# zeynelacikgoez/PyAudioLocalization

Measured on AMD Instinct MI355X. Metric: mic-pair GCC-PHAT correlations/s @44.1kHz·1s, higher is better.
Workload: dtype f64; 1 GPU; metric run: 64 frame(s)/step/GPU x 64 mics x 44100 samples @ 44100 Hz, 2016 pairs/frame, max_expected_delay=0.05; n=88199 = 89 x 991: prime-factor inverse, Rader row DFTs (cyclic convolutions of 990 points in LDS) + dense column DFTs; mics=64, samples=44100, pairs_per_frame=2016, fused_column_statistics=default, finishing_column_pass=default, rader_columns=default, gather=none, split=frames, parallelism=frames sharded over 1 GPU(s)

## Files before the change

pyaudiolocalization_amd/csrc/engine.h:

```cpp
#pragma once
#include <hip/hip_runtime.h>

#include <cstdarg>
#include <cstdint>
#include <cstdio>
#include <map>
#include <string>
#include <tuple>
#include <vector>

#include "../../include/pal_hip.h"
#include "fin_scratch.h"
#include "fft_core.h"
#include "pair_route.h"
#include "plan_geometry.h"
#include "peak_types.h"
#include "resample_math.h"

namespace pal {

struct FinArgs;

struct Conv {
  ConvGeom g;
// ... 179 lines not shown
  int solve_positions_dev(const pal_pair_record* d_tables, int B, int M, const int32_t* lengths, const double* mics, const double* calib,
                          const double* weights, const double* extra_starts, const pal_solve_params* prm, pal_position_record* out);
  int solve_positions_loss_dev(const pal_pair_record* d_tables, int B, int M, const int32_t* lengths, const double* mics, const double* calib,
                               const double* weights, const double* extra_starts, const pal_solve_params* prm, pal_position_record* out,
                               int loss, double f_scale, double* pair_weights);
  int solve_positions_impl(const pal_pair_record* d_tables, int B, int M, const int32_t* lengths, const double* mics, const double* calib,
                           const double* weights, const double* extra_starts, const pal_solve_params* prm, pal_position_record* out,
                           int loss, double f_scale, double* pair_weights);
  int tdoa_closure_dev(const pal_pair_record* d_tables, int B, int M, const int32_t* lengths, int32_t tol, int32_t min_votes, int32_t weight_mode,
                       int32_t* d_votes, int32_t* d_mic_closed, double* d_weights, pal_closure_frame* d_summary);
  int closure_check(int B, int M, const int32_t* lengths, int32_t tol, int32_t min_votes, int32_t weight_mode);
  int lag_votes(const int32_t* d_lag, int B, int M, int tol, int32_t* d_votes);
  int frames_check(const char* what, int B, int M, const int32_t* lengths, int32_t tol);
  int tdoa_consensus_dev(const pal_pair_record* d_tables, const int32_t* d_cand_k, const double* d_cand_h, int B, int M, int K,
                         const int32_t* lengths, int32_t tol, int32_t rounds, int32_t* d_sel, pal_pair_record* d_table_out,
                         pal_consensus_frame* d_summary);
  int consensus_check(int B, int M, int K, const int32_t* lengths, int32_t tol, int32_t rounds);
  int srp_strips_check(int B, int M, int L, int T, int W);
  int srp_strips_rows(const double* d_rows, int64_t nrows, int L, int T, int W, double* d_strips);
  int srp_map_check(int B, int M, int T, const double* mics, double fs, double c, const pal_srp_grid* grid, int K, int R, bool any_output,
                    bool peaks_out);
  int srp_map_dev(const double* d_strips, int B, int M, int T, const double* mics, double fs, double c, const pal_srp_grid* grid,
                  const double* d_pair_weights, int K, int R, double* d_power, pal_srp_peak* d_peaks, pal_srp_frame* d_summary);
  int srp_peaks_check(int B, const pal_srp_grid* grid, int K, int R);
  int srp_peaks_dev(const double* d_power, int B, const pal_srp_grid* grid, int K, int R, pal_srp_peak* d_peaks, pal_srp_frame* d_summary);
  int32_t* solve_idx = nullptr;
  int solve_idx_M = 0;
  std::vector<double> rs_win;
  std::vector<ResampleTap> rs_host;
  int rs_num_table = 0;
  double rs_ratio = 0;
  int peaks(const double* corr, size_t stride, int rows, int n, int n2, const pal_phat_params& prm,
            pal_pair_record* table, int32_t* ksel_multi, int slot, double* hsel_multi = nullptr);
  int peaks_setup(const double* corr, size_t stride, int rows, int n, int n2, const pal_phat_params& prm, int blocks, int grid_n2, int slot, PeakArgs& a);
  int peaks_finish(PeakArgs& a, int rows, pal_pair_record* table, int32_t* ksel_multi, int slot, double* hsel_multi = nullptr);
  int pfa_rows(const Plan& pl, const cd* permuted, const int4* quads, int G, cd* Y, hipStream_t on);
  int fin_setup(const Plan& pl, int rows, int nblk, int grid_rows, const pal_phat_params& prm, int n2, pal_pair_record* table,
                int* need, int slot, PeakArgs& a, struct FinArgs& fa, unsigned& nwg, int G);
  int rows_lean_group(const Plan& pl, const double* corr, size_t stride, int G, int rows, const pal_phat_params& prm, int n2,
                      pal_pair_record* table, int* need, int slot);
  int pfa_pair_group_fin(const Plan& pl, const cd* permuted, const int4* quads, int G, int rows, cd* Y, const int* zero_rows,
                         const pal_phat_params& prm, int n2, pal_pair_record* table, int* need, int slot,
                         double* corr = nullptr, size_t stride = 0);
  int pfa_pair_group_fused(const Plan& pl, const cd* permuted, const int4* quads, int G, int rows, cd* Y, double* corr, size_t stride,
                           const int* zero_rows, const pal_phat_params& prm, int n2, pal_pair_record* table, int32_t* ksel_multi, int slot,
                           double* hsel_multi = nullptr);
  bool pfa_forward_applies(const Plan& pl, int len) const;
  int pfa_forward_spectra(Plan& pl, const double* frames, size_t frame_stride, int rows, int len, cd* spectra, const int* flags);
  bool pfa_forward = true;
  bool fin_cols = true;
  unsigned fin_epoch[3] = {};
  FinKey fin_key[3];
  unsigned fin_wrap = kFinEpochWrap;
  bool fin_strip_on = true;
  int fin_giveup = 0;
  bool fuse_peaks = true;
};

struct ProfScope {
  Engine* e;
  int slot;
  hipEvent_t a = nullptr;
  hipStream_t on;
  ProfScope(Engine* eng, const char* name, hipStream_t s = nullptr) : e(eng), slot(-1), on(s ? s : eng->stream) {
    if (e->profiling && e->prof_gate) {
      slot = e->prof_slot(name);
      e->prof_begin(slot, &a, on);
    }
  }
  ~ProfScope() {
    if (slot >= 0) e->prof_end(slot, a, on);
  }
};

#define PAL_TRY(expr)                \
  do {                               \
    int _rc = (expr);                \
    if (_rc != PAL_OK) return _rc;   \
  } while (0)

#define PAL_HIP(expr) PAL_TRY(check((expr), #expr))

}
```

pyaudiolocalization_amd/csrc/pal_api.hip:

```cpp
#include <dlfcn.h>

#include <cmath>
#include <cstring>

#include "closure_tiles.h"
#include "engine.h"

namespace pal {

static std::string g_create_error;

int Engine::fail(int code, const char* fmt, ...) {
  char buf[512];
  va_list ap;
  va_start(ap, fmt);
  vsnprintf(buf, sizeof buf, fmt, ap);
  va_end(ap);
  err = buf;
  return code;
}

int Engine::check(hipError_t e, const char* what) {
  if (e == hipSuccess) return PAL_OK;
  const int code = e == hipErrorOutOfMemory ? PAL_ERR_NOMEM : PAL_ERR_HIP;
// ... 277 lines not shown
      (rc = hipEventCreateWithFlags(&e->ev_join2, hipEventDisableTiming)) != hipSuccess ||
      (rc = hipEventCreateWithFlags(&e->ev_join3, hipEventDisableTiming)) != hipSuccess ||
      (rc = hipEventCreateWithFlags(&e->ev_fin, hipEventDisableTiming)) != hipSuccess) {
    g_create_error = std::string("device init: ") + hipGetErrorString(rc);
    delete e;
    return PAL_ERR_HIP;
  }
  {
    int cus = 0;
    if (hipDeviceGetAttribute(&cus, hipDeviceAttributeMultiprocessorCount, device) == hipSuccess && cus > 0) e->cu_count = cus;
  }
  const char* env = getenv("PAL_CHUNK");
  if (env && atoi(env) > 0) { e->chunk = atoi(env); e->chunk_auto = false; }
  env = getenv("PAL_OVERLAP");
  e->one_stream = env && atoi(env) == 0;
  env = getenv("PAL_RADIX3");
  if (env) e->plan_sw.allow_r3 = atoi(env) != 0;
  env = getenv("PAL_PFA");
  if (env) e->plan_sw.allow_pfa = atoi(env) != 0;
  env = getenv("PAL_RADER");
  if (env) e->plan_sw.allow_rader = atoi(env) != 0;
  env = getenv("PAL_PFA_BIG");
  if (env) e->plan_sw.allow_big = atoi(env) != 0;
  env = getenv("PAL_FOUR_REG");
  if (env) e->plan_sw.four_reg = atoi(env) != 0;
  env = getenv("PAL_XCD_ROWS");
  if (env) e->xcd_rows = atoi(env) != 0;
  env = getenv("PAL_ROWS_SHARED");
  if (env) e->rows_shared = atoi(env) != 0;
  env = getenv("PAL_PFA_FWD");
  if (env) e->pfa_forward = atoi(env) != 0;
  env = getenv("PAL_FUSED");
  if (env) e->fuse_peaks = atoi(env) != 0;
  env = getenv("PAL_R89");
  if (env) e->plan_sw.allow_r89 = atoi(env) != 0;
  env = getenv("PAL_FIN_SERIAL");
  if (env) e->fin_serial = atoi(env) != 0;
  env = getenv("PAL_FIN");
  if (env) e->fin_cols = atoi(env) != 0;
  env = getenv("PAL_ROWS_LEAN");
  if (env) e->rows_lean = atoi(env) != 0;
  env = getenv("PAL_PAIR_BLOCK");
  if (env) e->pair_block = atoi(env);
  env = getenv("PAL_ROWS_LEAN_MIN");
  if (env && atoll(env) >= 1) e->rows_lean_min = atoll(env);
  env = getenv("PAL_LEAN_STORE");
  if (env) e->lean_store = atoi(env) != 0;
  env = getenv("PAL_DEBUG_MEMO");
  if (env) e->debug_memo = atoi(env);
  env = getenv("PAL_DEBUG_FIN_WRAP");
  if (env && atoi(env) >= 2) e->fin_wrap = unsigned(atoi(env));
  env = getenv("PAL_FIN_STRIP");
  if (env) e->fin_strip_on = atoi(env) != 0;
  env = getenv("PAL_DEBUG_FIN_GIVEUP");
  if (env) e->fin_giveup = atoi(env) != 0 ? 1 : 0;
  env = getenv("PAL_MAX_PLANS");
  if (env && atoi(env) >= 2) e->max_plans = atoi(env);
  *out = reinterpret_cast<pal_handle>(e);
  return PAL_OK;
}

void pal_destroy(pal_handle h) {
  if (!h) return;
  Engine* e = reinterpret_cast<Engine*>(h);
  hipSetDevice(e->device);
  pal_comm_destroy(h);
  (void)e->clear_plans();
  for (cd* p : e->stage_tw) if (p) hipFree(p);
  for (cd* p : e->stage_twc) if (p) hipFree(p);
  for (void* p : e->ws) if (p) hipFree(p);
  if (e->quads) hipFree(e->quads);
  if (e->quads_blk) hipFree(e->quads_blk);
  if (e->perm_blk) hipFree(e->perm_blk);
  if (e->solve_idx) hipFree(e->solve_idx);
  for (hipEvent_t ev : e->ev_pool) hipEventDestroy(ev);
  hipStreamDestroy(e->stream2);
  hipStreamDestroy(e->stream3);
  hipEventDestroy(e->ev_fork);
  hipEventDestroy(e->ev_join2);
  hipEventDestroy(e->ev_join3);
  hipEventDestroy(e->ev_fin);
  hipStreamDestroy(e->stream);
  delete e;
}

const char* pal_last_error(pal_handle h) {
  if (!h) return g_create_error.c_str();
  return reinterpret_cast<Engine*>(h)->err.c_str();
}

#define ENGINE(h)                                   \
  if (!(h)) return PAL_ERR_INVALID;                 \
  Engine* e = reinterpret_cast<Engine*>(h);         \
  if (hipSetDevice(e->device) != hipSuccess) return e->fail(PAL_ERR_HIP, "hipSetDevice(%d) failed", e->device)

int pal_synchronize(pal_handle h) {
  ENGINE(h);
  PAL_TRY(e->check(hipStreamSynchronize(e->stream), "stream sync"));
  if (e->profiling) e->prof_flush();
  return check_status(e);
}

int pal_clear_plans(pal_handle h) {
  ENGINE(h);
  return e->clear_plans();
}
// ... 639 lines not shown
```

pyaudiolocalization_amd/csrc/pfa.hip:

```cpp
#include <cmath>
#include <cstdlib>
#include <vector>

#include "pfa_kernels.h"
#include "pfa_rader.h"
#include "pfa_cols_stats.h"
#include "pfa_cols_fin.h"
#include "pfa_forward.h"
#include "pfa_big.h"

namespace pal {

#ifndef PAL_BIG13_PTS
#define PAL_BIG13_PTS 32
#endif
#ifndef PAL_BIG14_PTS
#define PAL_BIG14_PTS 32
#endif
constexpr int kBig13 = PAL_BIG13_PTS, kBig14 = PAL_BIG14_PTS;

static_assert(kColChunk == kPfaTC && kColUnroll == kPfaUnr && kRader89 == kR89, "plan_geometry.h against the column pass's constants");
static_assert(sizeof(RowStep) == sizeof(int2) && sizeof(Cplx) == sizeof(cd), "plan_geometry.h tables are uploaded as they are");

void Engine::free_pfa(Pfa& f) {
// ... 186 lines not shown
                      int* need, int slot, PeakArgs& a, FinArgs& fa, unsigned& nwg, int G) {
  const int n = pl.n;
  PAL_TRY(peaks_setup(nullptr, 0, rows, n, n2, prm, nblk, 0, slot, a));
  const FinLayout lay = fin_layout(pair_group(n), nblk, grid_rows);
  char* base = nullptr;
  PAL_TRY(scratch(fin_scratch_slot(slot), lay.total, &base));
  PAL_TRY(status_words(&fa.status));
  fa.table = table;
  fa.need = need;
  fa.done = reinterpret_cast<unsigned*>(base);
  FinKey key;
  key.gmax = pair_group(n);
  key.nblk = nblk;
  key.grid_rows = grid_rows;
  key.block = ws_bytes[fin_scratch_slot(slot)];
  if (fin_must_zero(fin_key[slot], key, fin_epoch[slot], fin_wrap)) {
    PAL_HIP(hipMemsetAsync(base, 0, key.block, stream_of(slot)));
    fin_key[slot] = key;
    fin_epoch[slot] = 0;
  }
  fa.epoch = ++fin_epoch[slot];
  fa.emax = reinterpret_cast<double*>(base + lay.off_emax);
  fa.parts = reinterpret_cast<FinPartial*>(base + lay.off_parts);
  fa.edge = reinterpret_cast<double*>(base + lay.off_edge);
  fa.giveup = fin_giveup;
  fa.pw = 1;
  fa.corr = nullptr;
  fa.stride = 0;
  fa.store_rows = 0;
  fa.strip = nullptr;
  fa.st = fin_no_strip();
  fa.grid = nullptr;
  fa.roots = nullptr;
  fa.zero_rows = nullptr;
  fa.windowed = std::isnan(prm.max_expected_delay) ? 0 : 1;
  fa.win_lo = 1;
  fa.win_hi = n - 2;
  if (fa.windowed) {
    const double med = prm.max_expected_delay, fs = prm.fs;
    long long k = -1;
    if (med >= 0) {
      const double est = med * fs;
      k = est < double(n) ? (long long)est + 2 : (long long)n;
      while (k >= 0 && !(std::fabs(double(k) / fs) <= med)) --k;
    }
    if (k < 0) { fa.win_lo = 1; fa.win_hi = 0; }
    else {
      const long long lo = (long long)(n2 - 1) - k, hi = (long long)(n2 - 1) + k;
      fa.win_lo = int(lo < 1 ? 1 : lo);
      fa.win_hi = int(hi > n - 2 ? n - 2 : hi);
    }
  }
  fa.cheb = a.method == 0 && nohist(prm.threshold_method, prm.threshold_multiplier) ? 1 : 0;
  nwg = 8u * unsigned((G + 7) / 8) * unsigned(nblk);
  return PAL_OK;
}

int Engine::rows_lean_group(const Plan& pl, const double* corr, size_t stride, int G, int rows, const pal_phat_params& prm, int n2,
                            pal_pair_record* table, int* need, int slot) {
  constexpr int NS = 22;
  const hipStream_t on = stream_of(slot);
  const int chunks = (pl.n + kColsOwn - 1) / kColsOwn;
  const int nblk = (chunks + 4 * NS - 1) / (4 * NS);
  PeakArgs a;
  FinArgs fa;
  unsigned nwg = 0;
  PAL_TRY(fin_setup(pl, rows, nblk, 1, prm, n2, table, need, slot, a, fa, nwg, G));
  fa.pw = 4;
  fa.corr = const_cast<double*>(corr);
  fa.stride = stride;
  ProfScope ps(this, "k_rows_lean", on);
  k_rows_lean<NS><<<dim3(nwg), dim3(256), 0, on>>>(corr, stride, G, nblk, a, fa, rows);
  PAL_HIP(hipGetLastError());
  return PAL_OK;
}

int Engine::pfa_pair_group_fin(const Plan& pl, const cd* permuted, const int4* quads, int G, int rows, cd* Y, const int* zero_rows,
                               const pal_phat_params& prm, int n2, pal_pair_record* table, int* need, int slot,
                               double* corr, size_t stride) {
  const Pfa& f = pl.pfa;
  const hipStream_t on = stream_of(slot);
  const bool shortcols = f.nch <= 1;
  const int nblk = fin_blocks(f.n2, f.nch);
  PeakArgs a;
  FinArgs fa;
  unsigned nwg = 0;
  PAL_TRY(fin_setup(pl, rows, nblk, f.n1, prm, n2, table, need, slot, a, fa, nwg, G));
  fa.corr = corr;
  fa.stride = stride;
  fa.store_rows = corr ? 1 : 0;
  PAL_TRY(pfa_rows(pl, permuted, quads, G, Y, on));
  {
    ProfScope ps(this, corr ? "k_pfa_cols_lean" : "k_pfa_cols_fin", on);
    const dim3 grid(nwg);
    const bool full = (f.n1 - 1) / 2 == f.nch * kPfaTC;
    const bool hist = !(a.method > 0 || fa.cheb);
    const int nw = f.nch == 2 ? 2 : (f.nch == 3 && !hist ? 3 : 4);
    FinSrc src{Y, f.T, static_cast<const Rader89Tab*>(f.r89_tab)};
    const FinStrip st = fin_strip(pl.n, fa.windowed != 0, fa.win_lo, fa.win_hi, a.snr_w, !corr && !hist, fin_strip_on);
    if (st.on()) {
      PAL_TRY(scratch(fin_strip_slot(slot), size_t(2 * pair_group(pl.n)) * size_t(st.len) * sizeof(double), &fa.strip));
      fa.st = st;
      fa.grid = Y;
      fa.roots = f.r1;
      fa.zero_rows = zero_rows;
    }
    const bool strip = fa.strip != nullptr;
    PAL_TRY(fin_serialize(on));
#define PAL_COLS_FIN(MODE, HI, FU, NW) do { \
      if (!HI && strip) k_pfa_cols_fin<MODE, kPfaTC, kPfaUnr, HI, FU, NW, !HI><<<grid, dim3(64 * NW), 0, on>>>(src, f.n1, f.n2, G, f.nch, nblk, zero_rows, a, fa, rows); \
      else k_pfa_cols_fin<MODE, kPfaTC, kPfaUnr, HI, FU, NW, false><<<grid, dim3(64 * NW), 0, on>>>(src, f.n1, f.n2, G, f.nch, nblk, zero_rows, a, fa, rows); } while (0)
#define PAL_COLS_FIN_FU(MODE, HI, NW) do { if (full) PAL_COLS_FIN(MODE, HI, true, NW); else PAL_COLS_FIN(MODE, HI, false, NW); } while (0)
    if (!hist) fa.pw = shortcols ? 4 : nw;
    if (shortcols) { if (hist) PAL_COLS_FIN(kColsStrips, true, false, 4); else PAL_COLS_FIN(kColsStrips, false, false, 4); }
    else if (f.r89 && full && nw == 4) { if (hist) PAL_COLS_FIN(kColsRader89, true, true, 4); else PAL_COLS_FIN(kColsRader89, false, true, 4); }
    else if (nw == 3) PAL_COLS_FIN_FU(kColsDense, false, 3);
    else if (nw == 2) { if (hist) PAL_COLS_FIN_FU(kColsDense, true, 2); else PAL_COLS_FIN_FU(kColsDense, false, 2); }
    else { if (hist) PAL_COLS_FIN_FU(kColsDense, true, 4); else PAL_COLS_FIN_FU(kColsDense, false, 4); }
#undef PAL_COLS_FIN_FU
#undef PAL_COLS_FIN
    PAL_HIP(hipGetLastError());
    PAL_TRY(fin_done(on));
  }
  return PAL_OK;
}

}
```

pyaudiolocalization_amd/csrc/pfa_cols_fin.h:

```cpp
#pragma once
#include <climits>

#include "fin_scratch.h"
#include "pair_route.h"
#include "pfa_cols_stats.h"
#include "reduce.h"
#include "wave_reduce.h"

namespace pal {

struct FinPartial {
  double vmin, hb, plat;
  double s1, s2, a1;
  double hw, platw;
  double hm;
  double w1, w2;
  int mb, mw, mm, pad;
};
static_assert(sizeof(FinPartial) == 104 && sizeof(FinPartial) == kFinPartialBytes, "thirteen words (fin_scratch.h)");

struct FinArgs {
  pal_pair_record* table;
  int* need;
  unsigned* done;
  double* edge;
  double* emax;
  unsigned epoch;
  int giveup;
  FinPartial* parts;
  int* status;
  int win_lo, win_hi;
  int windowed;
  int pw;
  double* corr;
  size_t stride;
  int store_rows;
  int cheb;
  double* strip;
  FinStrip st;
  const cd* grid;
  const cd* roots;
  const int* zero_rows;
};

struct FinWave {
  double vmax, hb, hw, hm, plat, platw, nvmin, s1, s2, a1, w1, w2;
  int imax, mb, mw, mm;
};

struct FinShared {
  unsigned hwin[2 * kWin];
  int swin0[144];
  FinWave wave[4];
};
static_assert(sizeof(FinShared) <= 2 * (kLogBins + 1) * sizeof(unsigned), "the finish scratch aliases the histograms");
// ... 250 lines not shown
      atomicAdd(&fs.hwin[kWin + 1], ld_agent(&bh[q].total));
    }
    for (int e = tid; e < S * kWin && have; e += LANES) {
      const int q = e / kWin, k = e - q * kWin;
      const int b = fs.swin0[q] + k;
      const unsigned v = ld_agent(&bh[q].h[k]);
      if (b < w0) atomicAdd(&fs.hwin[kWin], v);
      else if (b < wend) atomicAdd(&fs.hwin[b - w0], v);
    }
    __syncthreads();
    const unsigned total = fs.hwin[kWin + 1], base = fs.hwin[kWin];
    have = have && w0 < wend && total == unsigned(n) && r1 >= base;
    double b1lo = 0, b1hi = 0, b2lo = 0, b2hi = 0;
    if (have) {
      unsigned e = base;
      int f1 = -1, f2 = -1;
      for (int k = 0; k < wend - w0; ++k) {
        const unsigned v = fs.hwin[k];
        if (f1 < 0 && r1 < e + v) f1 = k;
        if (f2 < 0 && r2 < e + v) f2 = k;
        e += v;
      }
      have = f1 >= 0 && f2 >= 0;
      if (have) {
        b1lo = log_bin_floor(w0 + f1); b1hi = log_bin_floor(w0 + f1 + 1);
        b2lo = log_bin_floor(w0 + f2); b2hi = log_bin_floor(w0 + f2 + 1);
      }
    }
    __syncthreads();
    if (have) {
      const double ml_ = r2 != r1 ? (b1lo + b2lo) * 0.5 : b1lo, mh_ = r2 != r1 ? (b1hi + b2hi) * 0.5 : b1hi;
      tlo = pa.mult >= 0 ? pa.mult * ml_ : pa.mult * mh_;
      thi = pa.mult >= 0 ? pa.mult * mh_ : pa.mult * ml_;
    } else {
      flag = true;
      why |= 16;
    }
  }
  fin_decide(pa, fa, row, s, flag, why, interval, tlo, thi, tid == 0);
}

}
#include "pfa_fin_lean.h"
namespace pal {

enum { kColsDense = 0, kColsRader89 = 1, kColsStrips = 2 };

struct FinSrc {
  const cd* Y;
  const double* T;
  const Rader89Tab* tab;
};

template <int MODE, int TC, int UNR, bool HIST, bool FULL, int NW, bool STRIP = false>
__global__ __launch_bounds__(64 * NW) __attribute__((amdgpu_waves_per_eu(MODE == kColsRader89 ? 3 : 2))) void k_pfa_cols_fin(FinSrc src, int N1, int N2, int G, int nch, int nblk,
                                                      const int* __restrict__ zero_rows, PeakArgs pa, FinArgs fa, int rows) {
  constexpr bool R89 = MODE == kColsRader89, STRIPS = MODE == kColsStrips;
  static_assert(!R89 || (NW == 4 && FULL), "the Rader column transform is the four-wavefront N1 = 89 case");
  static_assert(!HIST || NW <= 4, "the histogram form merges at most four wavefronts per block");
  static_assert(!(HIST && STRIP), "the strip form belongs to the per-wavefront statistics");
  const cd* __restrict__ Y = src.Y;
  const double* __restrict__ T = src.T;
  const Rader89Tab* __restrict__ tab = src.tab;
  constexpr int kHistDoubles = (2 * (kLogBins + 1) * int(sizeof(unsigned)) + 7) / 8;
  __shared__ __attribute__((aligned(16))) double lds_big[R89 ? 88 * 64 : kHistDoubles];
  unsigned (*const hist)[kLogBins + 1] = reinterpret_cast<unsigned (*)[kLogBins + 1]>(lds_big);
  __shared__ FinPartial res[4][2];
  __shared__ double wmax[4][2];
  __shared__ unsigned wtot[4][2];
  __shared__ int medbin[2];
  __shared__ int s_imax[2];
  __shared__ int s_flag;
  const int tid = threadIdx.x, lane = tid & 63;
  const int wave = __builtin_amdgcn_readfirstlane(tid >> 6);
  const int ch = STRIPS ? 0 : wave;
  const int xs = int(blockIdx.x & 7u), slot = int(blockIdx.x >> 3);
  const int cb = slot % nblk, g = xs + 8 * (slot / nblk);
  if (g >= G) return;
  const int strips = STRIPS ? nblk * NW : nblk, strip = STRIPS ? cb * NW + wave : cb;
  const int nact = STRIPS ? NW : nch;
  const int c_lo = int((long long)strip * N2 / strips), c_hi = int((long long)(strip + 1) * N2 / strips);
  const bool active = STRIPS ? true : ch < nch;
  const int m2 = c_lo - 1 + lane;
  const bool live = m2 >= 0 && m2 < N2 && lane <= c_hi - c_lo + 1;
  const bool own = live && lane >= 1 && lane <= c_hi - c_lo;
  const bool inner = own && m2 >= 1 && m2 <= N2 - 2;
  const int m2c = m2 < 0 ? 0 : (m2 < N2 ? m2 : N2 - 1);
  const int h = (N1 - 1) / 2;
  const int n = pa.n;
  constexpr bool want_median = HIST;
  constexpr int LANES = 64 * NW;
  if (want_median && !R89) {
    unsigned* hz = &hist[0][0];
    for (int q = tid; q < 2 * (kLogBins + 1); q += LANES) hz[q] = 0;
  }
  constexpr int TCD = R89 ? 1 : TC;
  double cx[TCD], sy[TCD], cy[TCD], sx[TCD];
  double sumx = 0, sumy = 0;
  cd y0 = mk(0, 0);
  cd ro[R89 ? kR89Slots : 1];
  cd c0 = mk(0, 0);
  const double kp = zero_rows && zero_rows[2 * g] ? 0.0 : 1.0, kq = zero_rows && 2 * g + 1 < rows && zero_rows[2 * g + 1] ? 0.0 : 1.0;
  int slot_t = 0;
  if constexpr (R89) {
    slot_t = tab->tmap[wave][lane < kR89Slots ? lane : 0];
    r89_columns(Y + size_t(g) * N1 * N2 + m2c, N2, wave, lane, tab, lds_big, ro, c0);
    if (want_median) {
      unsigned* hz = &hist[0][0];
      for (int q = tid; q < 2 * (kLogBins + 1); q += LANES) hz[q] = 0;
    }
    if (kp == 0.0 || kq == 0.0) {
      c0.x *= kp; c0.y *= kq;
#pragma unroll
      for (int i = 0; i < kR89Slots; ++i) { ro[i].x *= kp; ro[i].y *= kq; }
    }
  } else {
    if (active) pfa_cols_accumulate<TC, UNR>(Y + size_t(g) * N1 * N2 + m2c, N1, N2, nch, ch, T, y0, cx, sy, cy, sx, sumx, sumy);
    if (kp == 0.0) { y0.x = sumx = 0.0; }
    if (kq == 0.0) { y0.y = sumy = 0.0; }
#pragma unroll
    for (int tt = 0; tt < TCD; ++tt) {
      cx[tt] *= kp; sy[tt] *= kp; cy[tt] *= kq; sx[tt] *= kq;
    }
  }
  if constexpr (!HIST) {
    bool last;
    if constexpr (R89) {
      last = fin_lean_r89<true, false, kR89Slots, STRIP>(ro, c0, slot_t, 0u, wave, lane, g, cb, nblk, N1, N2, rows, c_lo, m2, own, inner, cb == 0 || cb == nblk - 1,
                                                  -1, true, pa, fa);
    } else {
// ... 368 lines not shown
```

pyaudiolocalization_amd/csrc/pfa_fin_lean.h:

```cpp
#pragma once

namespace pal {

__device__ __forceinline__ double wave_max63r(double v) { return wave_reduce_d(v, -__builtin_huge_val(), [](double a, double b) { return max_raw(a, b); }); }
__device__ __forceinline__ double wave_min63r(double v) { return wave_reduce_d(v, __builtin_huge_val(), [](double a, double b) { return min_raw(a, b); }); }
__device__ __forceinline__ double readlane_d(double v, int l) {
  return __hiloint2double(__builtin_amdgcn_readlane(__double2hiint(v), l), __builtin_amdgcn_readlane(__double2loint(v), l));
}

template <class BETTER> __device__ __forceinline__ void uniform_arg_sparse(double& v, int& i, BETTER better) {
  const unsigned long long cm = __ballot(i >= 0);
  if (cm == 0) { i = -1; v = 0; return; }
  if ((cm & (cm - 1)) == 0) {
    const int l = int(__builtin_ctzll(cm));
    v = readlane_d(v, l);
    i = __builtin_amdgcn_readlane(i, l);
    return;
  }
  wave_arg63(v, i, better);
  v = wave_bcast63(v);
  i = wave_bcast63(i);
}
__device__ __forceinline__ void uniform_arg_dense_hi(double& v, int& i) {
  const double h = wave_bcast63(wave_max63r(i >= 0 ? v : -__builtin_huge_val()));
// ... 2 lines not shown
  if ((tm & (tm - 1)) == 0) {
    i = __builtin_amdgcn_readlane(i, int(__builtin_ctzll(tm)));
  } else {
    int j = (i >= 0 && v == h) ? i : -1;
    j = wave_reduce_i(j, -1, [](int a, int b) { return a > b ? a : b; });
    i = wave_bcast63(j);
  }
  v = h;
}
__device__ __forceinline__ void uniform_arg_dense_lo(double& v, int& i) {
  const double h = wave_bcast63(wave_max63r(i >= 0 ? v : -__builtin_huge_val()));
  const unsigned long long tm = __ballot(i >= 0 && v == h);
  if (tm == 0) { i = -1; v = 0; return; }
  if ((tm & (tm - 1)) == 0) {
    i = __builtin_amdgcn_readlane(i, int(__builtin_ctzll(tm)));
  } else {
    int j = (i >= 0 && v == h) ? i : INT_MAX;
    j = wave_reduce_i(j, INT_MAX, [](int a, int b) { return a < b ? a : b; });
    i = wave_bcast63(j);
  }
  v = h;
}
__device__ __forceinline__ double uniform_max_sparse(double v) {
  if (__ballot(v > -__builtin_huge_val()) == 0) return -__builtin_huge_val();
  return wave_bcast63(wave_max63r(v));
}

constexpr int kQuadXor1 = 0xB1, kQuadXor2 = 0x4E, kRor4 = 0x124, kRor8 = 0x128;
template <class OP> __device__ __forceinline__ double wave_pair_reduce(double a, double b, OP op) {
  const bool odd = threadIdx.x & 1;
  double c = odd ? b : a;
  const double d = odd ? a : b;
  c = op(c, dpp_d<kQuadXor1>(0.0, d));
  c = op(c, dpp_d<kQuadXor2>(0.0, c));
  c = op(c, dpp_d<kRor4>(0.0, c));
  c = op(c, dpp_d<kRor8>(0.0, c));
  {
    const unsigned lo = unsigned(__double2loint(c)), hi = unsigned(__double2hiint(c));
    const auto l = __builtin_amdgcn_permlane16_swap(lo, lo, false, false);
    const auto h = __builtin_amdgcn_permlane16_swap(hi, hi, false, false);
    c = op(__hiloint2double(int(h[0]), int(l[0])), __hiloint2double(int(h[1]), int(l[1])));
  }
  {
    const unsigned lo = unsigned(__double2loint(c)), hi = unsigned(__double2hiint(c));
    const auto l = __builtin_amdgcn_permlane32_swap(lo, lo, false, false);
    const auto h = __builtin_amdgcn_permlane32_swap(hi, hi, false, false);
    c = op(__hiloint2double(int(h[0]), int(l[0])), __hiloint2double(int(h[1]), int(l[1])));
  }
  return c;
}
__device__ __forceinline__ double wave_pair_sum(double a, double b) { return wave_pair_reduce(a, b, [](double x, double y) { return x + y; }); }
__device__ __forceinline__ double wave_pair_min(double a, double b) { return wave_pair_reduce(a, b, [](double x, double y) { return min_raw(x, y); }); }

template <bool ALL, bool PART, int NS, bool STRIP = false>
__device__ __forceinline__ bool fin_lean_r89(const cd (&ro)[NS], const cd c0, const int slot_t, const unsigned emask, const int wave, const int lane,
                                             const int g, const int cb, const int nblk, const int N1, const int N2, const int rows, const int c_lo,
                                             const int m2, const bool own, const bool inner, const bool edge_block, const int pslot, const bool pvalid,
                                             const PeakArgs& pa, const FinArgs& fa) {
  static_assert(NS + 1 <= 32, "slot masks are 32 bits");
  static_assert(!(STRIP && PART), "row chunks read stored rows: their finisher reads the SNR window from the row");
  const int n = pa.n, S = pa.splits, PW = fa.pw;
  const unsigned long long pvm = PART ? __ballot(pvalid) : ~0ull;
  const unsigned long long ownm = __ballot(own), innerm = __ballot(inner);
  const int nrow = 2 * g + 1 < rows ? 2 : 1;
  const bool windowed = fa.windowed != 0;
  auto T = [&](int slot) { return slot == 0 ? 0 : __builtin_amdgcn_readlane(slot_t, slot - 1); };
  auto for_slots = [&](int r, auto&& fn) {
    if (ALL ? wave == 0 : (emask & 1u) != 0) fn(r ? c0.y : c0.x, 0);
#pragma unroll
    for (int i = 0; i < NS; ++i)
      if (ALL || (emask >> (i + 1) & 1u)) fn(r ? ro[i].y : ro[i].x, i + 1);
  };
  auto slot_mask = [&](int t_lo, int t_hi) -> unsigned {
    const unsigned long long b = __ballot(lane < NS && slot_t >= t_lo && slot_t <= t_hi);
    const unsigned m = (unsigned(b) << 1) | (t_lo <= 0 && t_hi >= 0 ? 1u : 0u);
    return ALL ? (wave == 0 ? m : m & ~1u) : m & emask;
  };
  int lo1 = 1, hi1 = 0;
  unsigned wmask = 0;
  if (windowed) {
    const int elo = fa.win_lo - (pa.dist - 1), ehi = fa.win_hi + (pa.dist - 1);
    lo1 = elo > 1 ? elo : 1;
    hi1 = ehi < n - 2 ? ehi : n - 2;
    if (lo1 <= hi1) wmask = slot_mask(lo1 / N2, hi1 / N2);
  }

  double vn[2], s1[2], s2[2], a1[2];
  FinPartial pt[2];
#pragma unroll
  for (int r = 0; r < 2; ++r) {
    vn[r] = INFINITY; s1[r] = s2[r] = a1[r] = 0;
    pt[r].hb = 0; pt[r].plat = -INFINITY; pt[r].hw = 0; pt[r].platw = -INFINITY; pt[r].hm = 0;
    pt[r].mb = pt[r].mw = pt[r].mm = -1; pt[r].pad = 0;
    if (r >= nrow) continue;
    double vm = -INFINITY, vmin = INFINITY, t1 = 0, t2 = 0, ta = 0;
    for_slots(r, [&](double x, int slot) {
      if (PART && slot == pslot) {
        vm = pvalid ? max_raw(vm, x) : vm;
        vmin = pvalid ? min_raw(vmin, x) : vmin;
      } else {
        vm = max_raw(vm, x);
        vmin = min_raw(vmin, x);
      }
      t1 += x;
      t2 = __builtin_fma(x, x, t2);
      ta += fabs(x);
    });
    if (!own) { vm = -INFINITY; vmin = INFINITY; t1 = t2 = ta = 0; }
    vn[r] = vmin; s1[r] = t1; s2[r] = t2; a1[r] = ta;
    const double V = wave_bcast63(wave_max63r(vm));
    int im = INT_MAX, nhit = 0;
    bool vpeak = false;
    for_slots(r, [&](double x, int slot) {
      const unsigned long long mk = __ballot(x == V) & ownm & (PART && slot == pslot ? pvm : ~0ull);
      if (mk) {
        const int l = int(__builtin_ctzll(mk));
        const int cand = N2 * T(slot) + (c_lo - 1) + l;
        im = cand < im ? cand : im;
        nhit += __builtin_popcountll(mk);
        vpeak = (innerm >> l & 1ull) && (!PART || (cand >= 1 && cand <= n - 2)) && readlane_d(x, l - 1) < V && readlane_d(x, l + 1) < V;
      }
    });
    if (im == INT_MAX) im = -1;
    if (lane == 0)
      st_agent16(fa.emax + ((size_t(2 * g + r) * S + cb) * PW + wave) * 2, im >= 0 ? V : -INFINITY, double(fa.epoch) * kEpochUnit + double(im + 1));

    if (nhit == 1 && vpeak) {
      pt[r].hb = V; pt[r].mb = im; pt[r].plat = -INFINITY;
    } else {
#pragma nounroll
      for (int attempt = 0; attempt < 2; ++attempt) {
        const double pfloor = attempt == 0 && V > 0 ? 0.8 * V : -INFINITY;
        const double myfloor = inner ? pfloor : INFINITY;
        double hb = -INFINITY, plat = -INFINITY;
        int mb = -1;
        for_slots(r, [&](double x, int slot) {
          if (__ballot(x >= myfloor)) {
// ... 13 lines not shown
        if (mb >= 0 || pfloor == -INFINITY) break;
      }
    }
    if (wmask) {
      double hq = -INFINITY, hg = -INFINITY, platw = -INFINITY;
      int mq = -1, mg = -1;
      for_slots(r, [&](double x, int slot) {
        if (!(wmask >> slot & 1u)) return;
        const int m = m2 + N2 * T(slot);
        const double left = from_lower_lane(x), right = from_upper_lane(x);
        const bool in = inner && m >= lo1 && m <= hi1;
        platw = in && (left == x || right == x) ? fmax(platw, x) : platw;
        const bool pk = in && left < x && right < x;
        const bool inw = m >= fa.win_lo && m <= fa.win_hi;
        if (pk && inw && (x > hq || (x == hq && m > mq))) { hq = x; mq = m; }
        if (pk && !inw && (x > hg || (x == hg && m > mg))) { hg = x; mg = m; }
      });
      uniform_arg_dense_hi(hq, mq);
      uniform_arg_sparse(hg, mg, [](double v1, int i1, double v2, int i2) { return higher(v1, i1, v2, i2); });
      pt[r].hw = hq; pt[r].mw = mq; pt[r].hm = hg; pt[r].mm = mg;
      pt[r].platw = uniform_max_sparse(platw);
    }
  }

  if (edge_block) {
    const bool mine = own && (m2 <= 1 || m2 >= N2 - 2);
    if (__ballot(mine)) {
      const int e = m2 <= 1 ? m2 : 3 - (N2 - 1 - m2);
#pragma unroll
      for (int r = 0; r < 2; ++r) {
        if (r >= nrow) continue;
        double* dst = fa.edge + (size_t(2 * g + r) * 4 + (mine ? e : 0)) * N1;
        for_slots(r, [&](double x, int slot) {
          if (mine) st_agent(dst + T(slot), x);
        });
      }
    }
  }

  const bool stored = fa.corr != nullptr;
  if (stored && fa.store_rows) {
#pragma unroll
    for (int r = 0; r < 2; ++r) {
      if (r >= nrow) continue;
      double* const out = fa.corr + size_t(2 * g + r) * fa.stride + m2;
      for_slots(r, [&](double x, int slot) {
        const int t = T(slot);
        if (own && (!PART || N2 * t + m2 < n)) out[size_t(N2) * t] = x;
      });
    }
  }

  if constexpr (STRIP) {
    unsigned smask = 0;
#pragma unroll
    for (int p = 0; p < kFinStripPieces; ++p)
      if (p < fa.st.pieces) smask |= slot_mask(fa.st.lo[p] / N2, fa.st.hi[p] / N2);
    if (smask) {
#pragma unroll
      for (int r = 0; r < 2; ++r) {
        if (r >= nrow) continue;
        double* const dst = fa.strip + size_t(2 * g + r) * fa.st.len;
        for_slots(r, [&](double x, int slot) {
          if (!(smask >> slot & 1u)) return;
          const int off = fin_strip_offset(fa.st, m2 + N2 * T(slot));
          if (own && off >= 0) st_agent(dst + off, x);
        });
      }
    }
  }

  const double rmin = wave_pair_min(vn[0], vn[1]);
  const double r1 = wave_pair_sum(s1[0], s1[1]), r2 = wave_pair_sum(s2[0], s2[1]), ra = wave_pair_sum(a1[0], a1[1]);

  double w1[2] = {0, 0}, w2[2] = {0, 0};
  bool gave_up = false;
  bool have_w[2] = {false, false};
#pragma unroll
  for (int r = 0; r < 2; ++r) {
    if (STRIP || r >= nrow || stored) continue;
    const int row = 2 * g + r;
    double bv = -INFINITY;
    int bi = -1;
    const double* em = fa.emax + size_t(row) * S * PW * 2;
    const double want = double(fa.epoch);
    bool late = fa.giveup != 0;
    for (int q = lane; !fa.giveup && q < S * PW; q += 64) {
      double v = 0, code = 0;
      int spins = 0;
      for (;;) {
        ld_agent16(em + 2 * q, v, code);
        if (floor(code / kEpochUnit) == want) break;
        if (++spins > kSpinLimit) { late = true; break; }
        __builtin_amdgcn_s_sleep(8);
      }
      const int i = int(code - want * kEpochUnit) - 1;
      if (!late && i >= 0 && i < n && (bi < 0 || arg_better<0>(v, i, bv, bi))) { bv = v; bi = i; }
    }
    if (__ballot(late)) { gave_up = true; continue; }
    uniform_arg_dense_lo(bv, bi);
    int imax = bi;
    if (imax < 0 || imax >= n) imax = 0;
    const int A = imax - pa.snr_w > 0 ? imax - pa.snr_w : 0, B = imax + pa.snr_w < n ? imax + pa.snr_w : n;
    const int tA = A / N2, tB = (B - 1) / N2;
    const unsigned smask = slot_mask(tA, tB);
    if (smask == 0) continue;
    have_w[r] = true;
    const bool inA = m2 >= A - tA * N2, inB = m2 < B - tB * N2;
    double u1 = 0, u2 = 0;
    for_slots(r, [&](double x, int slot) {
// ... 170 lines not shown
```

pyaudiolocalization_amd/csrc/pfa_rader89.h:

```cpp
#pragma once
#include "fft_core.h"
#include "mixed_radix.h"

namespace pal {

constexpr int kR89 = 89;
constexpr int kR89Slots = 22;

struct Rader89Tab {
  int rowsel[4][24];
  int tmap[4][24];
  cd H[4][3][8];
};

PAL_HD int r89_crt(int b8, int b11) {
  return (33 * b8 + 56 * b11) % 88;
}

inline void make_rader89_tab(Rader89Tab& t) {
  const int g = 3, p = kR89;
  int gp[88], gm[88];
  long long x = 1;
  for (int a = 0; a < 88; ++a, x = x * g % p) gp[a] = int(x);
  for (int a = 0; a < 88; ++a) gm[a] = gp[(88 - a) % 88];
// ... 27 lines not shown

PAL_HD void r89_w8(int w, double& c, double& s) {
  const double h = 0.70710678118654752440;
  c = w == 0 ? 1.0 : (w == 1 ? h : (w == 2 ? 0.0 : -h));
  s = w == 0 ? 0.0 : (w == 2 ? 1.0 : h);
}

PAL_HD void r89_stage_a(cd* a, cd* b, int w) {
  dft_sym<11, false>(a);
  dft_sym<11, false>(b);
  double c, s;
  r89_w8(w, c, s);
#pragma unroll
  for (int k = 0; k < 11; ++k) {
    const cd sum = a[k] + b[k], dif = a[k] - b[k];
    a[k] = sum;
    b[k] = rotc<false>(dif, c, s);
  }
}

PAL_HD void r89_stage_b(cd* e, cd* o, const cd* H8, bool origin, cd y0, cd& c0) {
  dft4<false>(e);
  dft4<false>(o);
  if (origin) c0 = y0 + e[0];
#pragma unroll
  for (int q = 0; q < 4; ++q) {
    e[q] = cmul(e[q], H8[2 * q]);
    o[q] = cmul(o[q], H8[2 * q + 1]);
  }
  if (origin) e[0] = e[0] + y0;
  dft4<true>(e);
  dft4<true>(o);
}

PAL_HD void r89_stage_c(cd* z0, cd* z1, int w) {
  double c, s;
  r89_w8(w, c, s);
#pragma unroll
  for (int k = 0; k < 11; ++k) {
    const cd t = rotc<true>(z1[k], c, s);
    const cd p = z0[k] + t, m = z0[k] - t;
    z0[k] = p;
    z1[k] = m;
  }
  dft_sym<11, true>(z0);
  dft_sym<11, true>(z1);
}

}

#ifdef __HIPCC__
namespace pal {

__device__ __forceinline__ void r89_columns(const cd* __restrict__ Yg, int N2, int w, int lane, const Rader89Tab* __restrict__ tab,
                                            double* __restrict__ xch, cd* out, cd& c0) {
  const auto* rs = reinterpret_cast<const __attribute__((address_space(4))) int*>(reinterpret_cast<uintptr_t>(&tab->rowsel[w][0]));
  const auto* Hs = reinterpret_cast<const __attribute__((address_space(4))) double*>(reinterpret_cast<uintptr_t>(&tab->H[w][0][0]));
  cd v[22];
#pragma unroll
  for (int i = 0; i < 22; ++i) v[i] = Yg[size_t(rs[i]) * N2];
  const cd y0 = Yg[0];
  r89_stage_a(v, v + 11, w);
  cd e4[3][4], o4[3][4];
  double* const mine = xch + lane;
#pragma unroll
  for (int plane = 0; plane < 2; ++plane) {
#pragma unroll
    for (int i = 0; i < 22; ++i) mine[((w * 2 + i / 11) * 11 + i % 11) * 64] = plane ? v[i].y : v[i].x;
    __syncthreads();
#pragma unroll
    for (int q = 0; q < 3; ++q) {
      const int k11 = 3 * w + q < 11 ? 3 * w + q : 10;
#pragma unroll
      for (int ws = 0; ws < 4; ++ws) {
        const double a = mine[((ws * 2 + 0) * 11 + k11) * 64], b = mine[((ws * 2 + 1) * 11 + k11) * 64];
        if (plane) { e4[q][ws].y = a; o4[q][ws].y = b; } else { e4[q][ws].x = a; o4[q][ws].x = b; }
      }
    }
    __syncthreads();
  }
  c0 = mk(0, 0);
#pragma unroll
  for (int q = 0; q < 3; ++q) {
    cd H8[8];
#pragma unroll
    for (int k = 0; k < 8; ++k) H8[k] = mk(Hs[(q * 8 + k) * 2], Hs[(q * 8 + k) * 2 + 1]);
    cd c0q = mk(0, 0);
    r89_stage_b(e4[q], o4[q], H8, q == 0 && w == 0, y0, c0q);
    if (q == 0) c0 = c0q;
  }
#pragma unroll
  for (int plane = 0; plane < 2; ++plane) {
#pragma unroll
    for (int q = 0; q < 3; ++q) {
      const int k11 = 3 * w + q;
      if (k11 < 11) {
#pragma unroll
        for (int ws = 0; ws < 4; ++ws) {
          mine[((ws * 2 + 0) * 11 + k11) * 64] = plane ? e4[q][ws].y : e4[q][ws].x;
          mine[((ws * 2 + 1) * 11 + k11) * 64] = plane ? o4[q][ws].y : o4[q][ws].x;
        }
      }
    }
    __syncthreads();
#pragma unroll
    for (int i = 0; i < 22; ++i) {
      const double a = mine[((w * 2 + i / 11) * 11 + i % 11) * 64];
      if (plane) out[i].y = a; else out[i].x = a;
    }
    __syncthreads();
  }
  r89_stage_c(out, out + 11, w);
}

}
#endif
```

Baseline: 1.731 million pair-correlations/s.

## Add opt-in pipelined Rader-89 column finisher processing several blocks per workgroup

Adds a PIPE variant of the column-finish kernel where each workgroup walks K=4 consecutive column blocks, prefetching the next block's Rader-89 column inputs while transforming the current one, and computing slot masks once per workgroup. The goal is to hide global-load latency and amortise per-block setup, at the cost of fewer workgroups and lower occupancy. The path is gated behind PAL_FIN_PIPE, which defaults off. It also skips the unused q-slice for wave 3 in the Rader transform, which does run by default.

```diff
diff --git a/pyaudiolocalization_amd/csrc/engine.h b/pyaudiolocalization_amd/csrc/engine.h
--- a/pyaudiolocalization_amd/csrc/engine.h
+++ b/pyaudiolocalization_amd/csrc/engine.h
@@ -255,6 +255,7 @@
   unsigned fin_epoch[3] = {};
   FinKey fin_key[3];
   unsigned fin_wrap = kFinEpochWrap;
+  bool fin_pipe_on = false;
   bool fin_strip_on = true;
   int fin_giveup = 0;
   bool fuse_peaks = true;
diff --git a/pyaudiolocalization_amd/csrc/fin_pipe_items.h b/pyaudiolocalization_amd/csrc/fin_pipe_items.h
--- /dev/null
+++ b/pyaudiolocalization_amd/csrc/fin_pipe_items.h
@@ -0,0 +1,35 @@
+#pragma once
+
+#if defined(__HIPCC__) || defined(__CUDACC__)
+#define PAL_PIPE_HD __host__ __device__
+#else
+#define PAL_PIPE_HD
+#endif
+
+namespace pal {
+
+constexpr int kFinPipeBlocks = 4;
+
+struct FinPipeItem {
+  int stream;
+  int g;
+  int cb0, count;
+};
+
+PAL_PIPE_HD inline int fin_pipe_groups(int nblk, int K) { return (nblk + K - 1) / K; }
+
+PAL_PIPE_HD inline FinPipeItem fin_pipe_item(unsigned b, int nblk, int K) {
+  const int groups = fin_pipe_groups(nblk, K);
+  const int stream = int(b & 7u), slot = int(b >> 3);
+  const int grp = slot % groups;
+  FinPipeItem it;
+  it.stream = stream;
+  it.g = stream + 8 * (slot / groups);
+  it.cb0 = grp * K;
+  it.count = nblk - it.cb0 < K ? nblk - it.cb0 : K;
+  return it;
+}
+
+PAL_PIPE_HD inline unsigned fin_pipe_grid(int G, int nblk, int K) { return 8u * unsigned((G + 7) / 8) * unsigned(fin_pipe_groups(nblk, K)); }
+
+}
diff --git a/pyaudiolocalization_amd/csrc/pal_api.hip b/pyaudiolocalization_amd/csrc/pal_api.hip
--- a/pyaudiolocalization_amd/csrc/pal_api.hip
+++ b/pyaudiolocalization_amd/csrc/pal_api.hip
@@ -353,6 +353,8 @@
   if (env && atoi(env) >= 2) e->fin_wrap = unsigned(atoi(env));
   env = getenv("PAL_FIN_STRIP");
   if (env) e->fin_strip_on = atoi(env) != 0;
+  env = getenv("PAL_FIN_PIPE");
+  if (env) e->fin_pipe_on = atoi(env) != 0;
   env = getenv("PAL_DEBUG_FIN_GIVEUP");
   if (env) e->fin_giveup = atoi(env) != 0 ? 1 : 0;
   env = getenv("PAL_MAX_PLANS");
diff --git a/pyaudiolocalization_amd/csrc/pfa.hip b/pyaudiolocalization_amd/csrc/pfa.hip
--- a/pyaudiolocalization_amd/csrc/pfa.hip
+++ b/pyaudiolocalization_amd/csrc/pfa.hip
@@ -262,7 +262,7 @@
     }
   }
   fa.cheb = a.method == 0 && nohist(prm.threshold_method, prm.threshold_multiplier) ? 1 : 0;
-  nwg = 8u * unsigned((G + 7) / 8) * unsigned(nblk);
+  nwg = fin_pipe_grid(G, nblk, 1);
   return PAL_OK;
 }
 
@@ -322,11 +322,15 @@
       else k_pfa_cols_fin<MODE, kPfaTC, kPfaUnr, HI, FU, NW, false><<<grid, dim3(64 * NW), 0, on>>>(src, f.n1, f.n2, G, f.nch, nblk, zero_rows, a, fa, rows); } while (0)
 #define PAL_COLS_FIN_FU(MODE, HI, NW) do { if (full) PAL_COLS_FIN(MODE, HI, true, NW); else PAL_COLS_FIN(MODE, HI, false, NW); } while (0)
     if (!hist) fa.pw = shortcols ? 4 : nw;
+#define PAL_COLS_FIN_PIPE(K) k_pfa_cols_fin<kColsRader89, kPfaTC, kPfaUnr, false, true, 4, true, K><<<dim3(fin_pipe_grid(G, nblk, K)), dim3(256), 0, on>>>( \
+        src, f.n1, f.n2, G, f.nch, nblk, zero_rows, a, fa, rows)
     if (shortcols) { if (hist) PAL_COLS_FIN(kColsStrips, true, false, 4); else PAL_COLS_FIN(kColsStrips, false, false, 4); }
+    else if (f.r89 && full && nw == 4 && !hist && strip && fin_pipe_on) PAL_COLS_FIN_PIPE(kFinPipeBlocks);
     else if (f.r89 && full && nw == 4) { if (hist) PAL_COLS_FIN(kColsRader89, true, true, 4); else PAL_COLS_FIN(kColsRader89, false, true, 4); }
     else if (nw == 3) PAL_COLS_FIN_FU(kColsDense, false, 3);
     else if (nw == 2) { if (hist) PAL_COLS_FIN_FU(kColsDense, true, 2); else PAL_COLS_FIN_FU(kColsDense, false, 2); }
     else { if (hist) PAL_COLS_FIN_FU(kColsDense, true, 4); else PAL_COLS_FIN_FU(kColsDense, false, 4); }
+#undef PAL_COLS_FIN_PIPE
 #undef PAL_COLS_FIN_FU
 #undef PAL_COLS_FIN
     PAL_HIP(hipGetLastError());
diff --git a/pyaudiolocalization_amd/csrc/pfa_cols_fin.h b/pyaudiolocalization_amd/csrc/pfa_cols_fin.h
--- a/pyaudiolocalization_amd/csrc/pfa_cols_fin.h
+++ b/pyaudiolocalization_amd/csrc/pfa_cols_fin.h
@@ -1,6 +1,7 @@
 #pragma once
 #include <climits>
 
+#include "fin_pipe_items.h"
 #include "fin_scratch.h"
 #include "pair_route.h"
 #include "pfa_cols_stats.h"
@@ -357,13 +358,14 @@
   const Rader89Tab* tab;
 };
 
-template <int MODE, int TC, int UNR, bool HIST, bool FULL, int NW, bool STRIP = false>
-__global__ __launch_bounds__(64 * NW) __attribute__((amdgpu_waves_per_eu(MODE == kColsRader89 ? 3 : 2))) void k_pfa_cols_fin(FinSrc src, int N1, int N2, int G, int nch, int nblk,
+template <int MODE, int TC, int UNR, bool HIST, bool FULL, int NW, bool STRIP = false, int PIPE = 1>
+__global__ __launch_bounds__(64 * NW) __attribute__((amdgpu_waves_per_eu(PIPE > 1 ? 2 : (MODE == kColsRader89 ? 3 : 2)))) void k_pfa_cols_fin(FinSrc src, int N1, int N2, int G, int nch, int nblk,
                                                       const int* __restrict__ zero_rows, PeakArgs pa, FinArgs fa, int rows) {
   constexpr bool R89 = MODE == kColsRader89, STRIPS = MODE == kColsStrips;
   static_assert(!R89 || (NW == 4 && FULL), "the Rader column transform is the four-wavefront N1 = 89 case");
   static_assert(!HIST || NW <= 4, "the histogram form merges at most four wavefronts per block");
   static_assert(!(HIST && STRIP), "the strip form belongs to the per-wavefront statistics");
+  static_assert(PIPE == 1 || (R89 && STRIP), "several blocks per workgroup: Rader-89 columns, and nobody polls a sibling");
   const cd* __restrict__ Y = src.Y;
   const double* __restrict__ T = src.T;
   const Rader89Tab* __restrict__ tab = src.tab;
@@ -379,8 +381,47 @@
   const int tid = threadIdx.x, lane = tid & 63;
   const int wave = __builtin_amdgcn_readfirstlane(tid >> 6);
   const int ch = STRIPS ? 0 : wave;
-  const int xs = int(blockIdx.x & 7u), slot = int(blockIdx.x >> 3);
-  const int cb = slot % nblk, g = xs + 8 * (slot / nblk);
+  if constexpr (PIPE > 1) {
+    const FinPipeItem it = fin_pipe_item(blockIdx.x, nblk, PIPE);
+    const int g = it.g;
+    if (g >= G) return;
+    const double kp = zero_rows && zero_rows[2 * g] ? 0.0 : 1.0, kq = zero_rows && 2 * g + 1 < rows && zero_rows[2 * g + 1] ? 0.0 : 1.0;
+    const int slot_t = tab->tmap[wave][lane < kR89Slots ? lane : 0];
+    const FinSlotMasks sm = fin_slot_masks<true, kR89Slots>(slot_t, 0u, wave, lane, N2, pa, fa);
+    const cd* const Yg = Y + size_t(g) * N1 * N2;
+    auto column = [&](int cb) {
+      const int m2 = int((long long)cb * N2 / nblk) - 1 + lane;
+      return m2 < 0 ? 0 : (m2 < N2 ? m2 : N2 - 1);
+    };
+    cd v[kR89Slots], y0;
+    r89_load(Yg + column(it.cb0), N2, wave, tab, v, y0);
+    bool last = false;
+#pragma nounroll
+    for (int i = 0; i < it.count; ++i) {
+      const int cb = it.cb0 + i;
+      const int c_lo = int((long long)cb * N2 / nblk), c_hi = int((long long)(cb + 1) * N2 / nblk);
+      const int m2 = c_lo - 1 + lane;
+      const bool live = m2 >= 0 && m2 < N2 && lane <= c_hi - c_lo + 1;
+      const bool own = live && lane >= 1 && lane <= c_hi - c_lo;
+      const bool inner = own && m2 >= 1 && m2 <= N2 - 2;
+      cd ro[kR89Slots], c0;
+      r89_transform(v, y0, wave, lane, tab, lds_big, ro, c0);
+      if (i + 1 < it.count) r89_load(Yg + column(cb + 1), N2, wave, tab, v, y0);
+      if (kp == 0.0 || kq == 0.0) {
+        c0.x *= kp; c0.y *= kq;
+#pragma unroll
+        for (int k = 0; k < kR89Slots; ++k) { ro[k].x *= kp; ro[k].y *= kq; }
+      }
+      last = fin_lean_r89<true, false, kR89Slots, true>(ro, c0, slot_t, 0u, wave, lane, g, cb, nblk, N1, N2, rows, c_lo, m2, own, inner,
+                                                         cb == 0 || cb == nblk - 1, -1, true, pa, fa, &sm);
+    }
+    if (!last) return;
+    if (wave != 0) return;
+    fin_rows_wave<true>(pa, fa, g, nblk, rows, N1, N2, lane);
+    return;
+  }
+  const FinPipeItem item = fin_pipe_item(blockIdx.x, nblk, 1);
+  const int cb = item.cb0, g = item.g;
   if (g >= G) return;
   const int strips = STRIPS ? nblk * NW : nblk, strip = STRIPS ? cb * NW + wave : cb;
   const int nact = STRIPS ? NW : nch;
diff --git a/pyaudiolocalization_amd/csrc/pfa_fin_lean.h b/pyaudiolocalization_amd/csrc/pfa_fin_lean.h
--- a/pyaudiolocalization_amd/csrc/pfa_fin_lean.h
+++ b/pyaudiolocalization_amd/csrc/pfa_fin_lean.h
@@ -78,11 +78,40 @@
 __device__ __forceinline__ double wave_pair_sum(double a, double b) { return wave_pair_reduce(a, b, [](double x, double y) { return x + y; }); }
 __device__ __forceinline__ double wave_pair_min(double a, double b) { return wave_pair_reduce(a, b, [](double x, double y) { return min_raw(x, y); }); }
 
+template <bool ALL, int NS>
+__device__ __forceinline__ unsigned fin_slot_mask(int slot_t, unsigned emask, int wave, int lane, int t_lo, int t_hi) {
+  const unsigned long long b = __ballot(lane < NS && slot_t >= t_lo && slot_t <= t_hi);
+  const unsigned m = (unsigned(b) << 1) | (t_lo <= 0 && t_hi >= 0 ? 1u : 0u);
+  return ALL ? (wave == 0 ? m : m & ~1u) : m & emask;
+}
+__device__ __forceinline__ void fin_lag_span(const PeakArgs& pa, const FinArgs& fa, int& lo1, int& hi1) {
+  const int elo = fa.win_lo - (pa.dist - 1), ehi = fa.win_hi + (pa.dist - 1);
+  lo1 = elo > 1 ? elo : 1;
+  hi1 = ehi < pa.n - 2 ? ehi : pa.n - 2;
+}
+struct FinSlotMasks {
+  unsigned wmask;
+  unsigned smask;
+};
+template <bool ALL, int NS>
+__device__ __forceinline__ FinSlotMasks fin_slot_masks(int slot_t, unsigned emask, int wave, int lane, int N2, const PeakArgs& pa, const FinArgs& fa) {
+  FinSlotMasks sm{0u, 0u};
+  if (fa.windowed != 0) {
+    int lo1, hi1;
+    fin_lag_span(pa, fa, lo1, hi1);
+    if (lo1 <= hi1) sm.wmask = fin_slot_mask<ALL, NS>(slot_t, emask, wave, lane, lo1 / N2, hi1 / N2);
+  }
+#pragma unroll
+  for (int p = 0; p < kFinStripPieces; ++p)
+    if (p < fa.st.pieces) sm.smask |= fin_slot_mask<ALL, NS>(slot_t, emask, wave, lane, fa.st.lo[p] / N2, fa.st.hi[p] / N2);
+  return sm;
+}
+
 template <bool ALL, bool PART, int NS, bool STRIP = false>
 __device__ __forceinline__ bool fin_lean_r89(const cd (&ro)[NS], const cd c0, const int slot_t, const unsigned emask, const int wave, const int lane,
                                              const int g, const int cb, const int nblk, const int N1, const int N2, const int rows, const int c_lo,
                                              const int m2, const bool own, const bool inner, const bool edge_block, const int pslot, const bool pvalid,
-                                             const PeakArgs& pa, const FinArgs& fa) {
+                                             const PeakArgs& pa, const FinArgs& fa, const FinSlotMasks* const pre = nullptr) {
   static_assert(NS + 1 <= 32, "slot masks are 32 bits");
   static_assert(!(STRIP && PART), "row chunks read stored rows: their finisher reads the SNR window from the row");
   const int n = pa.n, S = pa.splits, PW = fa.pw;
@@ -98,17 +127,13 @@
       if (ALL || (emask >> (i + 1) & 1u)) fn(r ? ro[i].y : ro[i].x, i + 1);
   };
   auto slot_mask = [&](int t_lo, int t_hi) -> unsigned {
-    const unsigned long long b = __ballot(lane < NS && slot_t >= t_lo && slot_t <= t_hi);
-    const unsigned m = (unsigned(b) << 1) | (t_lo <= 0 && t_hi >= 0 ? 1u : 0u);
-    return ALL ? (wave == 0 ? m : m & ~1u) : m & emask;
+    return fin_slot_mask<ALL, NS>(slot_t, emask, wave, lane, t_lo, t_hi);
   };
   int lo1 = 1, hi1 = 0;
   unsigned wmask = 0;
   if (windowed) {
-    const int elo = fa.win_lo - (pa.dist - 1), ehi = fa.win_hi + (pa.dist - 1);
-    lo1 = elo > 1 ? elo : 1;
-    hi1 = ehi < n - 2 ? ehi : n - 2;
-    if (lo1 <= hi1) wmask = slot_mask(lo1 / N2, hi1 / N2);
+    fin_lag_span(pa, fa, lo1, hi1);
+    if (lo1 <= hi1) wmask = pre ? pre->wmask : slot_mask(lo1 / N2, hi1 / N2);
   }
 
   double vn[2], s1[2], s2[2], a1[2];
@@ -228,10 +253,10 @@
   }
 
   if constexpr (STRIP) {
-    unsigned smask = 0;
+    unsigned smask = pre ? pre->smask : 0u;
 #pragma unroll
     for (int p = 0; p < kFinStripPieces; ++p)
-      if (p < fa.st.pieces) smask |= slot_mask(fa.st.lo[p] / N2, fa.st.hi[p] / N2);
+      if (!pre && p < fa.st.pieces) smask |= slot_mask(fa.st.lo[p] / N2, fa.st.hi[p] / N2);
     if (smask) {
 #pragma unroll
       for (int r = 0; r < 2; ++r) {
diff --git a/pyaudiolocalization_amd/csrc/pfa_rader89.h b/pyaudiolocalization_amd/csrc/pfa_rader89.h
--- a/pyaudiolocalization_amd/csrc/pfa_rader89.h
+++ b/pyaudiolocalization_amd/csrc/pfa_rader89.h
@@ -103,14 +103,16 @@
 #ifdef __HIPCC__
 namespace pal {
 
-__device__ __forceinline__ void r89_columns(const cd* __restrict__ Yg, int N2, int w, int lane, const Rader89Tab* __restrict__ tab,
-                                            double* __restrict__ xch, cd* out, cd& c0) {
+__device__ __forceinline__ void r89_load(const cd* __restrict__ Yg, int N2, int w, const Rader89Tab* __restrict__ tab, cd (&v)[kR89Slots], cd& y0) {
   const auto* rs = reinterpret_cast<const __attribute__((address_space(4))) int*>(reinterpret_cast<uintptr_t>(&tab->rowsel[w][0]));
-  const auto* Hs = reinterpret_cast<const __attribute__((address_space(4))) double*>(reinterpret_cast<uintptr_t>(&tab->H[w][0][0]));
-  cd v[22];
 #pragma unroll
   for (int i = 0; i < 22; ++i) v[i] = Yg[size_t(rs[i]) * N2];
-  const cd y0 = Yg[0];
+  y0 = Yg[0];
+}
+
+__device__ __forceinline__ void r89_transform(cd (&v)[kR89Slots], const cd y0, int w, int lane, const Rader89Tab* __restrict__ tab,
+                                              double* __restrict__ xch, cd* out, cd& c0) {
+  const auto* Hs = reinterpret_cast<const __attribute__((address_space(4))) double*>(reinterpret_cast<uintptr_t>(&tab->H[w][0][0]));
   r89_stage_a(v, v + 11, w);
   cd e4[3][4], o4[3][4];
   double* const mine = xch + lane;
@@ -133,6 +135,7 @@
   c0 = mk(0, 0);
 #pragma unroll
   for (int q = 0; q < 3; ++q) {
+    if (3 * w + q >= 11) continue;
     cd H8[8];
 #pragma unroll
     for (int k = 0; k < 8; ++k) H8[k] = mk(Hs[(q * 8 + k) * 2], Hs[(q * 8 + k) * 2 + 1]);
@@ -164,5 +167,12 @@
   r89_stage_c(out, out + 11, w);
 }
 
+__device__ __forceinline__ void r89_columns(const cd* __restrict__ Yg, int N2, int w, int lane, const Rader89Tab* __restrict__ tab,
+                                            double* __restrict__ xch, cd* out, cd& c0) {
+  cd v[kR89Slots], y0;
+  r89_load(Yg, N2, w, tab, v, y0);
+  r89_transform(v, y0, w, lane, tab, xch, out, c0);
+}
+
 }
 #endif
```

Measured after the change: 1.738 million pair-correlations/s (median of 4 runs). About the same (+0.4%).
